# AtomGradient/swift-qwen3-tts

Hardware: AMD Instinct MI355X
Metric: codec_tokens_per_s (higher is better)
Workload: dtype bf16

## Files before the change

### swift-qwen3-tts_amd/csrc/engine.cc

```cpp
#include "engine.h"

#include <algorithm>
#include <cctype>
#include <chrono>
#include <cmath>
#include <cstdio>
#include <deque>
#include <functional>
#include <thread>

#include "codec.h"
#include "frontend.h"

namespace q3 {

namespace {
std::string lower(const std::string& s) {
    std::string o = s;
    for (auto& c : o) c = char(std::tolower((unsigned char)c));
    return o;
}
const char* const kCodecRangeMsg =
    "Audio decoding failed: the codec decoder produced a non-finite waveform -- also on the fp32 matrix-core convolutions (the "
    "reference's range), which a row is re-decoded on when it leaves the fp16 range of the default two-plane kernels";
// ... 27 lines not shown
    {
        int least = 0, greatest = 0;
        Q3_HIP(hipDeviceGetStreamPriorityRange(&least, &greatest));
        Q3_HIP(hipStreamCreateWithPriority(&st_, hipStreamNonBlocking, greatest));
        Q3_HIP(hipStreamCreateWithPriority(&st_codec_, hipStreamNonBlocking, least));
        hipDeviceProp_t prop{};
        Q3_HIP(hipGetDeviceProperties(&prop, m_->device));
        int cus = prop.multiProcessorCount / 2;
        if (opts.codec_overlap_cus > 0) cus = opts.codec_overlap_cus;
        else if (opts.codec_overlap_cus < 0) cus = 0;
        cus = std::min(cus, prop.multiProcessorCount) / 8 * 8;
        if (cus > 0 && cus < prop.multiProcessorCount) st_codec_part_ = masked_stream(cus, prop.multiProcessorCount);
    }
    for (auto& J : jobs_) {
        for (auto& e : J.ev_codec) Q3_HIP(hipEventCreate(&e));
        Q3_HIP(hipEventCreate(&J.ev_begin));
        Q3_HIP(hipEventCreate(&J.ev_first_audio));
        std::memset(J.nf_host.grow(size_t(std::max(opts.max_batch, 1))), 0, size_t(std::max(opts.max_batch, 1)) * 4);
    }
    for (auto& e : ev_) Q3_HIP(hipEventCreate(&e));
    for (auto& e : burst_ev_) Q3_HIP(hipEventCreateWithFlags(&e, hipEventDisableTiming));
    for (auto& e : ev_fe_) Q3_HIP(hipEventCreate(&e));
    Q3_HIP(hipEventCreateWithFlags(&fe_uploaded_, hipEventDisableTiming));
    Bm_ = opts.max_batch;
    Mp_ = std::getenv("Q3TTS_ROWS_64") ? 64 : std::max(256, 16 * int(align_up(size_t(opts.max_batch), 16)));
    Pcap_ = opts.max_prompt;
    Tcap_ = opts.max_prompt;
    Fcap_ = opts.max_frames;
    max_pages_ = ceil_div(Pcap_ + Fcap_ + 1, kPageTokens);
    n_pages_ = Bm_ * max_pages_;
    for (auto& kv : m_->cfg.talker.spk_id) speakers.push_back(kv.first);
    std::sort(speakers.begin(), speakers.end());
    alloc_workspace();
    if (std::getenv("Q3TTS_FRAME_STAMPS")) {
        Q3_HIP(hipMalloc(reinterpret_cast<void**>(&stamps_), 64 * 8));
        Q3_HIP(hipMemset(stamps_, 0, 64 * 8));
    }
    if (m_->has_codec) codec_ = std::make_unique<CodecRunner>(*m_, st_codec_, opts.codec_fp32 != 0);
    if (m_->has_codec_encoder || m_->has_speaker_encoder) fe_ = std::make_unique<VoiceFrontEnd>(*m_, st_);
}

hipStream_t Engine::masked_stream(int cus, int total) {
    std::vector<uint32_t> mask(size_t(ceil_div(total, 32)), 0u);
    for (int i = 0; i < cus; ++i) mask[size_t(i / 32)] |= 1u << (i % 32);
    hipStream_t st = nullptr;
    Q3_HIP(hipExtStreamCreateWithCUMask(&st, uint32_t(mask.size()), mask.data()));
    return st;
}

void Engine::prepare_job_pair() {
    job_chains = 2;
    if (opts_.codec_overlap_cus != 0 || !st_codec_part_ || st_codec_wide_) return;
    hipDeviceProp_t prop{};
    Q3_HIP(hipGetDeviceProperties(&prop, m_->device));
    st_codec_wide_ = masked_stream(prop.multiProcessorCount * 3 / 4 / 8 * 8, prop.multiProcessorCount);
}

Engine::~Engine() {
    if (worker_.joinable()) {
        {
            std::lock_guard<std::mutex> lk(work_mu_);
            work_stop_ = true;
        }
        work_cv_.notify_all();
        worker_.join();
    }
// ... 49 lines not shown
    if (st_) (void)hipStreamDestroy(st_);
}

void Engine::build_cp_proj_tables() {
    if (cp_tables_ || !m_->has_cp_proj || std::getenv("Q3TTS_NO_PROJ_TABLES")) return;
    const TalkerConfig& t = m_->cfg.talker;
    const int H = t.hidden_size, CH = m_->cp.hidden, MBL = Mp_ / 16, Vc = t.cp.vocab_size, nss = CH / 16;
    const int ntab = t.num_code_groups - 2;
    if (ntab <= 0) return;
    std::lock_guard<std::mutex> lock(m_->lazy_mutex);
    if (m_->cp_pe.empty()) {
        for (int i = 0; i < ntab; ++i) {
            uint16_t* pe = nullptr;
            float* pss = nullptr;
            Q3_HIP(hipMalloc(reinterpret_cast<void**>(&pe), size_t(Vc) * CH * 2));
            m_->lazy_allocs.push_back(pe);
            Q3_HIP(hipMalloc(reinterpret_cast<void**>(&pss), size_t(Vc) * nss * 4));
            m_->lazy_allocs.push_back(pss);
            for (int c0 = 0; c0 < Vc; c0 += Mp_) {
                const int rows = std::min(Mp_, Vc - c0);
                launch_tile_rows(m_->cp_emb[size_t(i)] + size_t(c0) * H, H, cp_x_, MBL, rows, H, st_);
                GemmArgs p = gemm_args(m_->cp_proj, cp_x_, rows);
                p.epi = 3; p.y = cp_.h; p.yMB = MBL; p.resid = 0; p.ss_out = cp_.ss_a;
                launch_gemm_skinny(p, st_);
                launch_untile_rows(cp_.h, MBL, pe + size_t(c0) * CH, CH, rows, CH, st_);
                launch_ss_to_table(cp_.ss_a, Mp_, pss + size_t(c0) * nss, nss, rows, st_);
            }
            m_->cp_pe.push_back(pe);
            m_->cp_pss.push_back(pss);
        }
        Q3_HIP(hipStreamSynchronize(st_));
    }
    cp_tables_ = true;
}

void Engine::alloc_workspace() {
    const TalkerConfig& t = m_->cfg.talker;
    const int H = t.hidden_size, CH = t.cp.hidden_size, TH = t.text_hidden_size;
    const int qd = t.num_attention_heads * kHeadDim, kd = t.num_key_value_heads * kHeadDim;
    const int cqd = t.cp.num_attention_heads * kHeadDim, ckd = t.cp.num_key_value_heads * kHeadDim;
    const int L = t.num_hidden_layers, CL = t.cp.num_hidden_layers;
    kv_layer_stride_ = size_t(n_pages_) * t.num_key_value_heads * kPageTokens * kHeadDim;
    cp_kv_layer_stride_ = size_t(Bm_) * t.cp.num_key_value_heads * kPageTokens * kHeadDim;
    proj_cap_ = Bm_ * (2 * Pcap_ + 8);
    for (int pass = 0; pass < 2; ++pass) {
        Bump b{pass ? ws_ : nullptr};
        Bump& x = b;
        auto stream = [&](Stream& s, int hid, int q, int k, int inter_p, int vocab) {
            s.ld_qkv = q + 2 * k;
            s.ld_act = inter_p;
            s.ld_logits = vocab;
            s.h = x.take<uint16_t>(size_t(Mp_) * hid);
            s.xn = x.take<uint16_t>(size_t(Mp_) * hid);
            s.ss_a = x.take<float>(size_t(hid / 16) * Mp_);
            s.ss_b = x.take<float>(size_t(hid / 16) * Mp_);
            s.qkv = x.take<uint16_t>(size_t(Mp_) * s.ld_qkv);
            s.ao = x.take<uint16_t>(size_t(Mp_) * q);
            s.act = x.take<uint16_t>(size_t(Mp_) * inter_p);
            s.logits = b.take<uint16_t>(size_t(Mp_) * vocab);
        };
        stream(tk_, H, qd, kd, m_->talker.max_inter_p, t.vocab_size);
        stream(cp_, CH, cqd, ckd, m_->cp.max_inter_p, t.cp.vocab_size);
        cp_x_ = x.take<uint16_t>(size_t(Mp_) * H);
        cp_x2_ = x.take<uint16_t>(size_t(Mp_) * H);
        cp_ss2_ = x.take<float>(size_t(Mp_));
        kpool_ = b.take<uint16_t>(kv_layer_stride_ * L);
// ... 20 lines not shown
        sp_dev_ = b.take<SamplingParams>(size_t(Bm_));
        ids_dev_ = b.take<int32_t>(size_t(proj_cap_));
        proj_in_ = b.take<uint16_t>(size_t(64) * TH);
        proj_mid_ = b.take<uint16_t>(size_t(64) * TH);
        proj_out_ = b.take<uint16_t>(size_t(proj_cap_ + 64) * H);
        compose_a_ = b.take<int32_t>(size_t(3) * Bm_ * (Pcap_ + Tcap_));
        compose_b_ = nullptr;
        if (!pass) {
            ws_bytes_ = align_up(b.off, 256);
            Q3_HIP(hipMalloc(reinterpret_cast<void**>(&ws_), ws_bytes_));
            Q3_HIP(hipMemset(ws_, 0, ws_bytes_));
        }
    }
    std::vector<int32_t> cbt((size_t)(Bm_));
    for (int i = 0; i < Bm_; ++i) cbt[size_t(i)] = i;
    Q3_HIP(hipMemcpy(cp_block_table_, cbt.data(), cbt.size() * 4, hipMemcpyHostToDevice));
}

GemmArgs Engine::gemm_args(const LinearW& L, const uint16_t* x, int M) const {
    GemmArgs a{};
    a.W = L.w;
    a.Wsb = L.sb;
    a.x = x;
    a.xMB = Mp_ / 16;
    a.M = M;
    a.Mpad = int(align_up(size_t(M), 16));
    a.N = L.Np;
    a.K = L.Kp;
    a.bias = L.bias;
    a.ss_ld = Mp_;
    return a;
}

void Engine::enqueue_layers(const StackW& s, Stream& w, int B, uint16_t* kpool, uint16_t* vpool, size_t layer_stride,
                            const int32_t* block_table, int max_pages, const int32_t* kv_len, const uint8_t* active,
                            int ss_count_in, int fixed_len, int chunk, const int32_t* chunk_n_prompt, int chunk_r_base) {
    const int H = s.hidden, MBL = Mp_ / 16, tiles = H / 16;
    const int M = B * (chunk > 1 ? chunk : 1);
    Q3_CHECK(M <= Mp_, 7, "internal error: chunk does not fit the activation buffers");
    const bool row_norm = M > 64;
    const bool prologue_qkv = H <= 2048 && !row_norm, prologue_mlp = H <= 2048 && !row_norm;
    const bool nt_off = debug_env().nt_off;
    const bool is_talker = &s == &m_->talker;
    const int ntw = is_talker && !nt_off ? 1 : 0;
    const int ntkv = ntw;
    auto norm_into_xn = [&](const uint16_t* nw, const float* ss, int ss_count) {
        NormRowsArgs n{};
        n.h = w.h; n.hMB = MBL; n.w = nw; n.eps = s.eps; n.out = w.xn; n.outMB = MBL; n.M = M; n.H = H;
        if (row_norm && H <= 2048) { n.ss_in = ss; n.ss_count = ss_count; n.ss_ld = Mp_; }
        launch_norm_rows(n, counted());
    };
    for (size_t l = 0; l < s.layers.size(); ++l) {
        const LayerW& L = s.layers[l];
        if (!prologue_qkv) norm_into_xn(L.ln1, w.ss_a, (l == 0) ? ss_count_in : tiles);
        GemmArgs q = gemm_args(L.qkv, prologue_qkv ? w.h : w.xn, M);
        q.epi = 0; q.y = w.qkv; q.ldy = w.ld_qkv; q.nt_weights = ntw;
        if (prologue_qkv) {
            q.norm_w = L.ln1; q.ss_in = w.ss_a; q.ss_count = (l == 0) ? ss_count_in : tiles; q.norm_dim = H; q.norm_eps = s.eps;
        }
        AttnArgs at{};
        at.qkv = w.qkv; at.ld = w.ld_qkv; at.qn_w = L.qn; at.kn_w = L.kn; at.eps = s.eps;
        at.rope_cos = s.rope_cos; at.rope_sin = s.rope_sin;
        at.kpool = kpool + l * layer_stride; at.vpool = vpool + l * layer_stride;
        at.block_table = block_table; at.max_pages = max_pages; at.kv_len = kv_len; at.active = active;
        at.out = w.ao; at.outMB = MBL; at.n_heads = s.n_heads; at.n_kv = s.n_kv; at.B = B;
        at.fixed_len = fixed_len; at.identity_pages = fixed_len >= 0 ? 1 : 0;
        at.chunk = chunk; at.chunk_n_prompt = chunk_n_prompt; at.chunk_r_base = chunk_r_base;
        at.scale = powf(float(kHeadDim), -0.5f);
        at.nt_kv = ntkv;
        launch_gemm_skinny(q, counted());
        launch_attn_decode(at, counted());
        GemmArgs o = gemm_args(L.o, w.ao, M);
        o.epi = 3; o.y = w.h; o.yMB = MBL; o.resid = 1; o.ss_out = w.ss_b; o.nt_weights = ntw;
        launch_gemm_skinny(o, counted());
        if (!prologue_mlp) norm_into_xn(L.ln2, w.ss_b, tiles);
        GemmArgs g = gemm_args(L.gateup, prologue_mlp ? w.h : w.xn, M);
        g.epi = 2; g.y = w.act; g.yMB = MBL; g.nt_weights = ntw;
        if (prologue_mlp) {
            g.norm_w = L.ln2; g.ss_in = w.ss_b; g.ss_count = tiles; g.norm_dim = H; g.norm_eps = s.eps;
        }
        launch_gemm_skinny(g, counted());
        GemmArgs d = gemm_args(L.down, w.act, M);
        d.epi = 3; d.y = w.h; d.yMB = MBL; d.resid = 1; d.ss_out = w.ss_a; d.nt_weights = ntw;
        launch_gemm_skinny(d, counted());
    }
}

void Engine::enqueue_talker_step(int B, bool with_head) {
    (void)with_head;
    enqueue_layers(m_->talker, tk_, B, kpool_, vpool_, kv_layer_stride_, block_table_, max_pages_, kv_len_, active_, 1, -1, 1, nullptr, 0);
}

void Engine::enqueue_cp_pass(int B, bool from_talker, int head, int cp_pos, bool projected) {
    const TalkerConfig& t = m_->cfg.talker;
    const int H = t.hidden_size, CH = m_->cp.hidden, MBL = Mp_ / 16;
    int ss_count = 1;
    auto talker_norm_into = [&](uint16_t* dst, float* ss_out) {
        NormRowsArgs n{};
        n.h = tk_.h; n.hMB = MBL; n.w = m_->talker.final_norm; n.eps = m_->talker.eps;
        n.out = dst; n.outMB = MBL; n.ss_out = ss_out; n.M = B; n.H = H;
        launch_norm_rows(n, counted());
    };
    if (m_->has_cp_proj && projected) {
        ss_count = CH / 16;
    } else if (m_->has_cp_proj) {
        if (from_talker) talker_norm_into(cp_x2_, nullptr);
        GemmArgs p = gemm_args(m_->cp_proj, from_talker ? cp_x2_ : cp_x_, B);
        p.epi = 3; p.y = cp_.h; p.yMB = MBL; p.resid = 0; p.ss_out = cp_.ss_a;
        launch_gemm_skinny(p, counted());
        ss_count = CH / 16;
    } else if (from_talker) {
        talker_norm_into(cp_.h, cp_.ss_a);
    }
    enqueue_layers(m_->cp, cp_, B, cp_kpool_, cp_vpool_, cp_kv_layer_stride_, cp_block_table_, 1, cp_len_, nullptr, ss_count, cp_pos, 1, nullptr, 0);
}

void Engine::enqueue_frame(int B, const DebugOpts* dbg) {
    struct Count {
        Engine* e;
        int B;
        ~Count() { e->frame_launches_[B] = e->launches_; }
    } count{this, B};
    launches_ = 0;
    const TalkerConfig& t = m_->cfg.talker;
    const int H = t.hidden_size, V = t.vocab_size, Vc = t.cp.vocab_size, CH = t.cp.hidden_size;
    const int groups = t.num_code_groups, MBL = Mp_ / 16;
    stamp(0);
    enqueue_talker_step(B, true);
    stamp(1);
    uint16_t* next_x = m_->has_cp_proj ? cp_x_ : cp_.h;
    float* next_ss = m_->has_cp_proj ? nullptr : cp_.ss_a;
    const bool pair = 2 * B <= Mp_;
    {
        GemmArgs hd = gemm_args(m_->codec_head, tk_.h, B);
        hd.epi = 0; hd.y = tk_.logits; hd.ldy = tk_.ld_logits;
        hd.norm_w = m_->talker.final_norm; hd.ss_in = tk_.ss_a; hd.ss_count = H / 16; hd.norm_dim = H; hd.norm_eps = m_->talker.eps;
        bool rode = false;
        if (pair) {
            NormRowsArgs n{};
            n.h = tk_.h; n.hMB = MBL; n.w = m_->talker.final_norm; n.eps = m_->talker.eps;
            n.out = next_x; n.outMB = MBL; n.ss_out = next_ss; n.M = B; n.H = H;
            rode = launch_gemm_skinny_with_norm_rows(hd, n, st_);
            if (rode) ++launches_;
            else launch_norm_rows(n, counted());
        }
        if (!rode) launch_gemm_skinny(hd, counted());
    }
// ... 14 lines not shown
    sa.logits_dump = (dbg && dbg->talker_logits) ? tl_dump_ : nullptr; sa.dump_ld = V; sa.dump_off = 0;
    sa.row_key = frame_row_key_;
    if (pair) {
        launch_sampler(sa, counted());
        int ss_count = 1;
        if (m_->has_cp_proj) {
            GemmArgs p = gemm_args(m_->cp_proj, cp_x_, 2 * B);
            p.epi = 3; p.y = cp_.h; p.yMB = MBL; p.resid = 0; p.ss_out = cp_.ss_a;
            launch_gemm_skinny(p, counted());
            ss_count = CH / 16;
        }
        stamp(2);
        enqueue_layers(m_->cp, cp_, B, cp_kpool_, cp_vpool_, cp_kv_layer_stride_, cp_block_table_, 1, cp_len_, nullptr, ss_count, 0, 2,
                       nullptr, 0);
        stamp(3);
    } else {
        launch_sampler(sa, counted());
        enqueue_cp_pass(B, true, -1, 0);
        if (!m_->has_cp_proj) {
            launch_copy_rows(cp_x2_, 0, cp_.h, 0, 1, Mp_ * H, counted());
            launch_copy_rows(reinterpret_cast<const uint16_t*>(cp_ss2_), 0, reinterpret_cast<uint16_t*>(cp_.ss_a), 0, 1, Mp_ * 2, counted());
        }
    }
    FrameEndArgs fe{};
    fe.cur_codes = cur_codes_; fe.codec_emb = m_->codec_emb; fe.cp_emb = m_->cp_emb_dev;
    fe.trailing = trailing_; fe.n_trailing = n_trailing_; fe.trailing_idx = trailing_idx_; fe.Tmax = Tcap_;
    fe.tts_pad = tts_pad_; fe.h = tk_.h; fe.hMB = MBL; fe.ss_out = tk_.ss_a; fe.H = H; fe.B = B; fe.groups = groups;
    fe.n_frames = n_frames_; fe.max_frames = max_frames_; fe.finished = finished_; fe.active = active_; fe.cp_len = cp_len_;
    bool fe_done = false;
    for (int i = 0; i < groups - 1; ++i) {
        const bool second_of_pair = pair && i == 0;
        const int Mh = second_of_pair ? 2 * B : B;
        if (!second_of_pair) {
            enqueue_cp_pass(B, false, i, i + 1, cp_tables_ && i >= 1);
            stamp(5);
        }
        {
            GemmArgs lh = gemm_args(m_->lm_head[size_t(i)], cp_.h, Mh);
            lh.epi = 0; lh.y = cp_.logits; lh.ldy = cp_.ld_logits;
            lh.norm_w = m_->cp.final_norm; lh.ss_in = cp_.ss_a; lh.ss_count = CH / 16; lh.norm_dim = CH; lh.norm_eps = m_->cp.eps;
            launch_gemm_skinny(lh, counted());
        }
        SamplerArgs sc{};
        sc.logits = cp_.logits + (second_of_pair ? size_t(B) * cp_.ld_logits : 0); sc.ldl = cp_.ld_logits; sc.V = Vc; sc.sp = sp_dev_;
        sc.is_talker = 0;
        sc.eos_id = -1; sc.cb = i + 1; sc.n_frames = n_frames_; sc.max_frames = max_frames_;
        sc.finished = finished_; sc.active = active_; sc.kv_len = cp_len_; sc.advance = 1; sc.advance_gate = nullptr;
        sc.cur_codes = cur_codes_; sc.codes = codes_; sc.Fmax = Fcap_;
        sc.forced = dbg ? forced_dev_ : nullptr; sc.forced_frames = dbg ? dbg->frames : 0;
        sc.sampled = dbg ? sampled_dev_ : nullptr;
        if (i + 1 < groups - 1) {
            sc.emb = m_->cp_emb[size_t(i)]; sc.emb_ld = H; sc.next_x = next_x; sc.next_MB = MBL; sc.next_ss = next_ss;
        }
        sc.H = H; sc.B = B;
        if (cp_tables_ && i + 1 < groups - 1) {
            sc.emb = m_->cp_pe[size_t(i)]; sc.emb_ld = CH; sc.H = CH; sc.next_x = cp_.h;
            sc.emb_ss = m_->cp_pss[size_t(i)]; sc.nss = CH / 16; sc.next_ss = cp_.ss_a; sc.next_ss_ld = Mp_;
        }
        sc.logits_dump = (dbg && dbg->cp_logits) ? cl_dump_ : nullptr; sc.dump_ld = (groups - 1) * Vc; sc.dump_off = i * Vc;
        sc.row_key = frame_row_key_;
        if (i == groups - 2 && Vc <= 2048) {
            launch_sampler_with_frame_end(sc, fe, counted());
            fe_done = true;
        } else {
            launch_sampler(sc, counted());
        }
        stamp(second_of_pair ? 4 : 6);
    }
    if (!fe_done) launch_frame_end(fe, counted());
    stamp(7);
}

hipGraphExec_t Engine::frame_graph(int B) {
    std::map<int, hipGraphExec_t>& graphs = frame_row_key_ ? qgraphs_ : graphs_;
    auto it = graphs.find(B);
    if (it != graphs.end()) return it->second;
    hipGraph_t g = nullptr;
    Q3_HIP(hipStreamBeginCapture(st_, hipStreamCaptureModeThreadLocal));
    try {
        enqueue_frame(B, nullptr);
    } catch (...) {
        (void)hipStreamEndCapture(st_, &g);
        if (g) (void)hipGraphDestroy(g);
        throw;
    }
    Q3_HIP(hipStreamEndCapture(st_, &g));
    hipGraphExec_t ge = nullptr;
    Q3_HIP(hipGraphInstantiate(&ge, g, nullptr, nullptr, 0));
    Q3_HIP(hipGraphDestroy(g));
    graphs[B] = ge;
// ... 888 lines not shown
    Q3_HIP(hipMemsetAsync(seen_, 0, size_t(n) * m_->cfg.talker.vocab_size, st_));
    Q3_HIP(hipMemsetAsync(codes_, 0, size_t(n) * Fcap_ * 16 * 4, st_));
    upload_sampling(sp, row_offset + sp.row_base, n);
    return Pmax;
}

void Engine::debug_buffers(int n, const DebugOpts& dbg) {
    const TalkerConfig& t = m_->cfg.talker;
    const int V = t.vocab_size, Vc = t.cp.vocab_size;
    for (void* p : {(void*)forced_dev_, (void*)sampled_dev_, (void*)tl_dump_, (void*)cl_dump_})
        if (p) (void)hipFree(p);
    forced_dev_ = sampled_dev_ = nullptr;
    tl_dump_ = cl_dump_ = nullptr;
    const size_t nf = size_t(n) * dbg.frames;
    if (dbg.forced_codes) {
        for (size_t i = 0; i < nf * 16; ++i) {
            const int32_t c = dbg.forced_codes[i];
            Q3_CHECK(c >= 0 && c < ((i & 15) == 0 ? V : Vc), 3, "Invalid input: forced code outside its vocabulary");
        }
        Q3_HIP(hipMalloc(reinterpret_cast<void**>(&forced_dev_), nf * 16 * 4));
        Q3_HIP(hipMemcpy(forced_dev_, dbg.forced_codes, nf * 16 * 4, hipMemcpyHostToDevice));
    }
    Q3_HIP(hipMalloc(reinterpret_cast<void**>(&sampled_dev_), nf * 16 * 4));
    Q3_HIP(hipMemset(sampled_dev_, 0xff, nf * 16 * 4));
    if (dbg.talker_logits) Q3_HIP(hipMalloc(reinterpret_cast<void**>(&tl_dump_), nf * V * 2));
    if (dbg.cp_logits) Q3_HIP(hipMalloc(reinterpret_cast<void**>(&cl_dump_), nf * (t.num_code_groups - 1) * Vc * 2));
}

int Engine::frame_loop(Job& J, const std::vector<ResolvedRequest>& rr, const q3tts_sampling& sp, q3tts_event_cb cb, void* user,
                       const DebugOpts* dbg, StreamedDecode& sd) {
    const int n = J.n;
    const bool use_graph = opts_.use_graph && !dbg;
    build_cp_proj_tables();
    hipGraphExec_t ge = use_graph ? frame_graph(n) : nullptr;
    int frames_cap = 0;
    for (auto& r : rr) frames_cap = std::max(frames_cap, r.max_frames);
    std::vector<int32_t> h_nframes((size_t)(n), 0);
    std::vector<uint8_t> h_fin((size_t)(n), 0);
    std::vector<int> reported((size_t)(n), 0);
    int launched = 0;
    const bool fixed_len = sp.force_frames > 0 || dbg;
    const int burst_frames = std::max(1, max_inflight_frames / job_chains / 2);
    hipEvent_t ring[2] = {burst_ev_[0], burst_ev_[1]};
    int bursts = 0;
    bool done = false;
    while (!done && launched < frames_cap) {
        if (bursts >= 2) Q3_HIP(hipEventSynchronize(ring[bursts & 1]));
        int burst = std::min(burst_frames, frames_cap - launched);
        if (sd.on) {
            const int need = std::min(frames_cap, sd.next_need(launched, sp.audio_chunk_frames, std::max(0, sp.audio_lookahead_frames)));
            if (need > launched) burst = std::min(burst, need - launched);
        }
        for (int i = 0; i < burst; ++i) {
            if (use_graph) Q3_HIP(hipGraphLaunch(ge, st_));
            else enqueue_frame(n, dbg);
        }
        launched += burst;
        if (!(fixed_len && !cb)) {
            Q3_HIP(hipMemcpyAsync(h_nframes.data(), n_frames_, size_t(n) * 4, hipMemcpyDeviceToHost, st_));
            Q3_HIP(hipMemcpyAsync(h_fin.data(), finished_, size_t(n), hipMemcpyDeviceToHost, st_));
        }
        Q3_HIP(hipEventRecord(ring[bursts & 1], st_));
        ++bursts;
        if (fixed_len && !cb) {
            if (sd.on) {
                for (int b = 0; b < n; ++b) sd.avail[size_t(b)] = std::min(launched, rr[size_t(b)].max_frames);
// ... 653 lines not shown
    launch_admit_rows(a, k, st_);
    Q3_HIP(hipEventRecord(ev_[1], st_));
    const double now = now_s();
    for (int j = 0; j < k; ++j) {
        sl[size_t(slots[size_t(j)])] = QSlot{idx[size_t(j)], 0, 0, np[size_t(j)], now, rr[size_t(j)].max_frames};
        live[idx[size_t(j)]].rr = std::move(rr[size_t(j)]);
    }
    return k;
}

void Engine::run_queued(QueueShared& q, int S, const q3tts_sampling& sp, q3tts_event_cb cb, void* user) {
    Q3_HIP(hipSetDevice(m_->device));
    Q3_CHECK(S >= 1 && S <= Bm_, 3, "Invalid input: slots must be between 1 and max_batch");
    Q3_CHECK(!job_outstanding(), 3, "Invalid input: a q3tts_generate_begin job is outstanding (q3tts_generate_end must be called first)");
    ensure_queue_ws();
    {
        if (q.voice_ref_max >= 0) extra_.grow(size_t(S) * (1 + q.voice_ref_max) * m_->cfg.talker.hidden_size);
    }
    const double t_call = now_s();
    std::vector<int32_t> bt(size_t(S) * max_pages_);
    for (size_t i = 0; i < bt.size(); ++i) bt[i] = int32_t(i);
    Q3_HIP(hipMemcpyAsync(block_table_, bt.data(), bt.size() * 4, hipMemcpyHostToDevice, st_));
    for (int32_t* p : {kv_len_, cp_len_, n_frames_, max_frames_, trailing_idx_, n_trailing_, n_prompt_})
        Q3_HIP(hipMemsetAsync(p, 0, size_t(S) * 4, st_));
    Q3_HIP(hipMemsetAsync(row_key_, 0, size_t(S) * 4, st_));
    Q3_HIP(hipMemsetAsync(active_, 0, size_t(S), st_));
    Q3_HIP(hipMemsetAsync(finished_, 1, size_t(S), st_));
    {
        q3tts_sampling call_wide = sp;
        call_wide.per_request = nullptr;
        upload_sampling(call_wide, 0u, S);
    }
    build_cp_proj_tables();
    struct KeyScope {
        Engine* e;
        ~KeyScope() { e->frame_row_key_ = nullptr; }
    } key_scope{this};
    frame_row_key_ = row_key_;
    hipGraphExec_t ge = opts_.use_graph ? frame_graph(S) : nullptr;
    Q3_HIP(hipStreamSynchronize(st_));

    std::vector<QSlot> sl((size_t)(S));
    std::unordered_map<int, QLive> live;
    std::vector<int> settled;
    std::deque<int> waiting;
    int dec = -1;
    struct DecodeGuard {
        Engine* e;
        int* dec;
        ~DecodeGuard() {
            if (*dec < 0) return;
            (void)hipEventSynchronize(e->jobs_[*dec].ev_codec[1]);
            e->release_job(e->jobs_[*dec]);
        }
    } dec_guard{this, &dec};
    double codec_ms = 0;
    auto deliver = [&](bool wait) {
        if (!wait) {
            std::lock_guard<std::mutex> lk(stage_mu_);
            if (jobs_[dec].stage == 1) return;
        }
        const int j = dec;
        dec = -1;
        const std::vector<int> batch = jobs_[j].req_index;
        end(j, nullptr);
        codec_ms += timing.codec_ms;
// ... 1268 lines not shown
```

### swift-qwen3-tts_amd/csrc/engine.h

```cpp
#pragma once
#include <atomic>
#include <cstdlib>
#include <map>
#include <memory>
#include <condition_variable>
#include <mutex>
#include <thread>
#include <string>
#include <unordered_map>
#include <vector>

#include "../../include/q3tts.h"
#include "kernels.h"
#include "model.h"
#include "session_queue.h"

namespace q3 {

struct DebugOpts {
    const int32_t* forced_codes = nullptr;
    int frames = 0;
    uint16_t* talker_logits = nullptr;
    uint16_t* cp_logits = nullptr;
    int32_t* sampled = nullptr;
// ... 162 lines not shown
    Model* m_;
  public:
    uint32_t row_offset = 0;
    std::mutex* cb_mutex = nullptr;
    int request_base = 0;
    int max_inflight_frames = 16;
    int job_chains = 1;
  private:
    q3tts_load_opts opts_;
    hipStream_t st_ = nullptr;
    hipStream_t st_codec_ = nullptr;
    hipStream_t st_codec_part_ = nullptr;
    hipStream_t st_codec_wide_ = nullptr;
    hipStream_t masked_stream(int cus, int total);
    hipStream_t codec_stream(bool overlapped, bool wide = false);
    hipEvent_t ev_[4] = {nullptr, nullptr, nullptr, nullptr};
    hipEvent_t burst_ev_[2] = {nullptr, nullptr};
    hipEvent_t ev_fe_[2] = {nullptr, nullptr};
    hipEvent_t fe_uploaded_ = nullptr;
    int Bm_ = 0, Mp_ = 0;
    int Pcap_ = 0, Tcap_ = 0, Fcap_ = 0, max_pages_ = 0, n_pages_ = 0;

    uint8_t* ws_ = nullptr;
    size_t ws_bytes_ = 0;
    struct Stream {
        uint16_t *h, *xn, *qkv, *ao, *act, *logits;
        float *ss_a, *ss_b;
        int ld_qkv, ld_act, ld_logits;
    } tk_{}, cp_{};
    uint16_t* cp_x_ = nullptr;
    uint16_t* cp_x2_ = nullptr;
    bool cp_tables_ = false;
    void build_cp_proj_tables();
    float* cp_ss2_ = nullptr;
    uint16_t *kpool_ = nullptr, *vpool_ = nullptr, *cp_kpool_ = nullptr, *cp_vpool_ = nullptr;
    size_t kv_layer_stride_ = 0, cp_kv_layer_stride_ = 0;
    int32_t *block_table_ = nullptr, *cp_block_table_ = nullptr;
    int32_t *kv_len_ = nullptr, *cp_len_ = nullptr, *n_frames_ = nullptr, *max_frames_ = nullptr;
    int32_t *trailing_idx_ = nullptr, *n_trailing_ = nullptr, *n_prompt_ = nullptr, *cur_codes_ = nullptr, *codes_ = nullptr;
    uint8_t *active_ = nullptr, *finished_ = nullptr, *seen_ = nullptr;
    uint16_t *prompt_ = nullptr, *trailing_ = nullptr, *tts_pad_ = nullptr;
    SamplingParams* sp_dev_ = nullptr;
    int32_t* ids_dev_ = nullptr;
    uint16_t *proj_in_ = nullptr, *proj_mid_ = nullptr, *proj_out_ = nullptr;
    int proj_cap_ = 0;
    int32_t *compose_a_ = nullptr, *compose_b_ = nullptr;
    int32_t *forced_dev_ = nullptr, *sampled_dev_ = nullptr;
    uint16_t *tl_dump_ = nullptr, *cl_dump_ = nullptr;

    struct Job {
        std::atomic<bool> busy{false};
        uint64_t seq = 0;
        std::vector<ResolvedRequest> rr;
        std::vector<int> np;
        q3tts_sampling sp{};
        bool overlapped = false;
        bool frontend = false;
        bool background = false;
        int back = 0;
        int back_status = 0;
        std::string back_err;
        int n = 0, Fdec = 0, up = 0;
        std::vector<int> frames, ref_T, target_tokens, n_prompt;
        std::vector<int> req_index;
        std::vector<q3tts_result*> row_out;
        std::vector<double> row_span;
// ... 73 lines not shown
    const float* upload_audio(const float* audio, int64_t n);
    bool prepare_clone_rows(std::vector<ResolvedRequest>& reqs);

    void alloc_workspace();
    ResolvedRequest resolve(const q3tts_request& r, const q3tts_sampling& sp, const Voice* voice = nullptr) const;
    void check_reference(const float* ref_audio, int64_t n_ref_samples, const int32_t* ref_text_ids, int n_ref_text_ids) const;
    int open_job(const q3tts_request* reqs, int n, const q3tts_sampling& sp, const DebugOpts* dbg, std::vector<ResolvedRequest>& rr,
                 double& t_start, const Voice* const* voices);
    int reserve_rows(const std::vector<ResolvedRequest>& rr, const std::vector<int>& np, const std::vector<int>& nt,
                     const q3tts_sampling& sp);
    void debug_buffers(int n, const DebugOpts& dbg);
    struct StreamedDecode;
    struct SlotStream;
    int frame_loop(Job& J, const std::vector<ResolvedRequest>& rr, const q3tts_sampling& sp, q3tts_event_cb cb, void* user,
                   const DebugOpts* dbg, StreamedDecode& sd);
    void hand_off(Job& J, const std::vector<ResolvedRequest>& rr, StreamedDecode& sd, int launched, bool overlapped);
    void back_half(Job& J, const std::vector<ResolvedRequest>& rr, const std::vector<int>& np, const q3tts_sampling& sp,
                   q3tts_event_cb cb, void* user, const DebugOpts* dbg, bool streamed, bool overlapped, double t_start);
    void worker_loop();
    std::thread worker_;
    std::mutex work_mu_;
    std::condition_variable work_cv_;
    Job* work_ = nullptr;
    bool work_stop_ = false;
    void job_timing(Job& J, const std::vector<int>& np, int launched);
    void upload_sampling(const q3tts_sampling& sp, uint32_t row0, int n);
    int64_t kv_bytes(int n_prompt, int frames) const;
    int launches_per_step(int B) const;
    void assemble_prompts(const std::vector<ResolvedRequest>& reqs, std::vector<int>& n_prompt, std::vector<int>& n_trailing,
                          const std::vector<int>* trailing_rows = nullptr);
    void enqueue_prefill(Stream& w, int n, int Pmax, const int32_t* block_table, int32_t* kv_len, const int32_t* n_prompt,
                         uint8_t* active);
    void project_rows(const std::vector<int32_t>& ids, int rows);
    void enqueue_layers(const StackW& s, Stream& w, int B, uint16_t* kpool, uint16_t* vpool, size_t layer_stride,
                        const int32_t* block_table, int max_pages, const int32_t* kv_len, const uint8_t* active,
                        int ss_count_in, int fixed_len, int chunk, const int32_t* chunk_n_prompt, int chunk_r_base);
    void enqueue_talker_step(int B, bool with_head);
    void enqueue_cp_pass(int B, bool from_talker, int head, int cp_pos, bool projected = false);
    void enqueue_frame(int B, const DebugOpts* dbg);
    hipGraphExec_t frame_graph(int B);
    const uint32_t* frame_row_key_ = nullptr;
    std::map<int, hipGraphExec_t> qgraphs_;
    uint8_t* qws_ = nullptr;
    Stream qk_{};
    int32_t *q_bt_ = nullptr, *q_kv_len_ = nullptr, *q_n_prompt_ = nullptr;
    uint8_t* q_active_ = nullptr;
    AdmitDesc* q_desc_ = nullptr;
    std::vector<AdmitDesc> q_desc_host_;
    uint32_t* row_key_ = nullptr;
    std::vector<int32_t> q_host_;
    void ensure_queue_ws();
    struct QSlot {
        int req = -1;
        int since = 0;
        int reported = 0;
        int np = 0;
        double t0 = 0;
        int cap = 0;
    };
    struct QLive;
    int admit(QueueShared& q, std::vector<QSlot>& sl, std::unordered_map<int, QLive>& live);
    void cancel_slots(uint64_t mask, int slots);
    GemmArgs gemm_args(const LinearW& L, const uint16_t* x, int M) const;
};


class Session;

class EngineGroup {
  public:
    EngineGroup(std::unique_ptr<Model> model, const q3tts_load_opts& opts);
// ... 90 lines not shown
```

### swift-qwen3-tts_amd/csrc/kernels.h

```cpp
#pragma once
#include <hip/hip_runtime.h>

#include <cstdint>

namespace q3 {

struct DebugEnv {
    bool gemm_no_row_split;
    bool gemm_one_pair;
    bool no_tall_gemm;
    int tall_shape;
    int chunk_qsplit;
    bool conv_no_pw;
    bool nt_off;
    bool serial_jobs;
    bool fail_back_half;
    bool no_prefix_cache;
};
const DebugEnv& debug_env();
void debug_env_reload();

constexpr int kPageTokens = 64;
constexpr int kHeadDim = 128;

// ... 106 lines not shown
    const uint16_t* logits;
    int ldl, V;
    const SamplingParams* sp;
    int is_talker;
    int suppress_lo, suppress_hi, eos_id;
    uint8_t* seen;
    int cb;
    const int32_t* n_frames;
    const int32_t* max_frames;
    uint8_t* finished;
    uint8_t* active;
    int32_t* kv_len;
    int advance;
    const uint8_t* advance_gate;
    int32_t* cur_codes;
    int32_t* codes;
    int Fmax;
    const int32_t* forced;
    int forced_frames;
    int32_t* sampled;
    const uint16_t* emb;
    int emb_ld;
    uint16_t* next_x;
    int next_MB;
    int next_row0;
    float* next_ss;
    const float* emb_ss;
    int nss, next_ss_ld;
    int H;
    int B;
    uint16_t* logits_dump;
    int dump_ld, dump_off;
    const uint32_t* row_key;
};
void launch_sampler(const SamplerArgs& a, hipStream_t st);
void launch_sampler_with_frame_end(const SamplerArgs& a, const FrameEndArgs& fe, hipStream_t st);
void launch_ss_to_table(const float* ss, int ss_ld, float* dst, int nss, int rows, hipStream_t st);

void launch_gather_rows(const uint16_t* table, int ld, const int32_t* ids, const int32_t* token_map,
                        int n, int dim, uint16_t* out, int ldo, int out_MB, hipStream_t st);
void launch_tile_rows(const uint16_t* src, int lds, uint16_t* dst, int dstMB, int rows, int dim, hipStream_t st);
void launch_untile_rows(const uint16_t* src, int srcMB, uint16_t* dst, int ldd, int rows, int dim, hipStream_t st);
void launch_add_rows(const uint16_t* a, int lda, const uint16_t* b, int ldb, int rows, int dim,
                     uint16_t* out, int ldo, hipStream_t st);

struct PrefillLoadArgs {
    const uint16_t* prompt;
    const int32_t* n_prompt;
    int Pmax, step, H, B;
    uint16_t* h;
    int hMB;
    float* ss_out;
    uint8_t* active;
};
void launch_prefill_load(const PrefillLoadArgs& a, hipStream_t st);
void launch_advance_len(int32_t* kv_len, const uint8_t* active, int B, hipStream_t st);
void launch_stamp(unsigned long long* acc, unsigned long long* last, int k, hipStream_t st);
void launch_prefill_chunk_load(const PrefillLoadArgs& a, int C, hipStream_t st);
void launch_advance_len_chunk(int32_t* kv_len, const int32_t* n_prompt, int r_base, int C, int B, hipStream_t st);

struct AdmitDesc {
    int32_t slot, n_trailing, max_frames;
    uint32_t row_key;
    SamplingParams sp;
};
struct AdmitArgs {
    const AdmitDesc* desc;
    const uint16_t* src_h;
// ... 35 lines not shown
```

### swift-qwen3-tts_amd/csrc/kernels/sampler.hip

```cpp
#include "../common.h"
#include "../kernels.h"
#include "row_jobs.h"

namespace q3 {
namespace {

constexpr int kMaxVAll = 4096;

__device__ __forceinline__ void philox4x32_10(uint32_t c0, uint32_t c1, uint32_t c2, uint32_t c3, uint32_t k0,
                                              uint32_t k1, uint32_t (&out)[4]) {
#pragma unroll
    for (int r = 0; r < 10; ++r) {
        const uint64_t p0 = (uint64_t)0xD2511F53u * c0;
        const uint64_t p1 = (uint64_t)0xCD9E8D57u * c2;
        const uint32_t n0 = (uint32_t)(p1 >> 32) ^ c1 ^ k0;
        const uint32_t n1 = (uint32_t)p1;
        const uint32_t n2 = (uint32_t)(p0 >> 32) ^ c3 ^ k1;
        const uint32_t n3 = (uint32_t)p0;
        c0 = n0; c1 = n1; c2 = n2; c3 = n3;
        k0 += 0x9E3779B9u;
        k1 += 0xBB67AE85u;
    }
    out[0] = c0; out[1] = c1; out[2] = c2; out[3] = c3;
}
// ... 75 lines not shown
        float a, b, c, d;
        if constexpr (O == 32) { XorPartner::swap32(x.v, a, b); XorPartner::swap32(fi, c, d); }
        else { XorPartner::swap16(x.v, a, b); XorPartner::swap16(fi, c, d); }
        const bool upper = O == 32 ? ((threadIdx.x & 32) != 0) : ((threadIdx.x & 16) != 0);
        y.v = upper ? a : b;
        y.i = __float_as_int(upper ? c : d);
    } else if constexpr (O == 8) {
        y.v = XorPartner::x8(x.v); y.i = __float_as_int(XorPartner::x8(fi));
    } else if constexpr (O == 4) {
        y.v = XorPartner::x4(x.v); y.i = __float_as_int(XorPartner::x4(fi));
    } else if constexpr (O == 2) {
        y.v = XorPartner::x2(x.v); y.i = __float_as_int(XorPartner::x2(fi));
    } else {
        y.v = XorPartner::x1(x.v); y.i = __float_as_int(XorPartner::x1(fi));
    }
    return y;
}

template <int kThreads>
__device__ Best block_argmax(Best x, Best* scratch) {
    x = better(x, partner<32>(x));
    x = better(x, partner<16>(x));
    x = better(x, partner<8>(x));
    x = better(x, partner<4>(x));
    x = better(x, partner<2>(x));
    x = better(x, partner<1>(x));
    const int wave = threadIdx.x >> 6;
    __syncthreads();
    if ((threadIdx.x & 63) == 0) scratch[wave] = x;
    __syncthreads();
    Best r = scratch[0];
    for (int w = 1; w < kThreads / 64; ++w) r = better(r, scratch[w]);
    return r;
}

template <int kThreads, int kMaxV, bool TALKER, bool FEND>
__device__ __forceinline__ void sampler_body(const SamplerArgs& a, const FrameEndArgs* fe) {
    constexpr int kElems = kMaxV / kThreads;
    __builtin_amdgcn_s_setprio(3);
    __shared__ float vals[kMaxV];
    __shared__ uint32_t sortbuf[kMaxV];
    __shared__ float sval[kMaxV];
    __shared__ int n_surv;
    __shared__ uint32_t hist[2][256];
    __shared__ Best scratch[kThreads / 64];
    __shared__ uint32_t wcount[kElems][kThreads / 64];
    __shared__ int sel[2][2];

    const int b = blockIdx.x, tid = threadIdx.x;
    const int V = a.V;
    const uint16_t* lrow = a.logits + (size_t)b * a.ldl;
    uint16_t raw[kElems];
    uint8_t was_seen[kElems];
    const bool want_seen = TALKER && a.seen;
#pragma unroll
    for (int k = 0; k < kElems; ++k) {
        const int i = k * kThreads + tid;
        const int ic = i < V ? i : V - 1;
        raw[k] = lrow[ic];
        was_seen[k] = want_seen ? a.seen[(size_t)b * V + ic] : (uint8_t)0;
    }
    const SamplingParams sp = a.sp[b];
    const bool row_done = a.finished[b] != 0;
    const int frame = a.n_frames[b];
    const uint8_t gate_raw = *(a.advance_gate ? a.advance_gate + b : a.finished + b);
    const uint32_t key_raw = *(a.row_key ? a.row_key + b : reinterpret_cast<const uint32_t*>(a.n_frames) + b);
// ... 192 lines not shown
            }
        }
        __syncthreads();
        const int ns = n_surv;
        Best x{-INFINITY, 0x7fffffff};
        for (int q = tid; q < ns; q += kThreads) {
            const int i = (int)sortbuf[q];
            const float v = rbf(sval[q] * invt) + gumbel_noise(sp.seed, row_key, draw, (uint32_t)i);
            x = better(x, Best{v, i});
        }
        Best r = block_argmax<kThreads>(x, scratch);
        tok = (r.i == 0x7fffffff) ? 0 : r.i;
    }

    int used = tok;
    if (a.forced && frame < a.forced_frames) used = a.forced[((size_t)b * a.forced_frames + frame) * 16 + a.cb];
    if (tid == 0) {
        if (a.sampled && frame < a.forced_frames) a.sampled[((size_t)b * a.forced_frames + frame) * 16 + a.cb] = tok;
        a.cur_codes[(size_t)b * 16 + a.cb] = used;
        if (TALKER) {
            if (a.seen && used >= 0 && used < V) a.seen[(size_t)b * V + used] = 1;
            if (a.advance && a.active[b]) a.kv_len[b] += 1;
            if (used == a.eos_id) {
                a.finished[b] = 1;
                a.active[b] = 0;
            } else if (frame < a.Fmax) {
                a.codes[((size_t)b * a.Fmax + frame) * 16] = used;
            }
        } else {
            if (a.advance && gate) a.kv_len[b] += 1;
            if (frame < a.Fmax) a.codes[((size_t)b * a.Fmax + frame) * 16 + a.cb] = used;
        }
    }
    if (a.next_x) {
        const uint4* src = reinterpret_cast<const uint4*>(a.emb + (size_t)used * a.emb_ld);
        float ss = 0.f;
        for (int i = tid; i < a.H / 8; i += kThreads) {
            const uint4 v = src[i];
            const uint32_t w[4] = {v.x, v.y, v.z, v.w};
#pragma unroll
            for (int j = 0; j < 4; ++j) ss += lo_bf(w[j]) * lo_bf(w[j]) + hi_bf(w[j]) * hi_bf(w[j]);
            *reinterpret_cast<uint4*>(a.next_x + act_tiled_offset(b + a.next_row0, 8 * i, a.next_MB)) = v;
        }
        if (a.emb_ss) {
            for (int j = tid; j < a.nss; j += kThreads)
                a.next_ss[(size_t)j * a.next_ss_ld + b + a.next_row0] = a.emb_ss[(size_t)used * a.nss + j];
        } else if (a.next_ss) {
            ss = wave_sum(ss);
            __syncthreads();
            if ((tid & 63) == 0) vals[tid >> 6] = ss;
            __syncthreads();
            if (tid == 0) {
                float t = 0.f;
                for (int w = 0; w < kThreads / 64; ++w) t += vals[w];
                a.next_ss[b] = t;
            }
        }
    }
    if constexpr (FEND) {
        __shared__ float fe_sh[4];
        frame_end_job(*fe, b, tid, used, fe_sh);
    }
}

template <int kThreads, int kMaxV, bool TALKER>
__global__ __launch_bounds__(kThreads) void sampler_kernel(SamplerArgs a) {
    sampler_body<kThreads, kMaxV, TALKER, false>(a, nullptr);
}
struct SamplerFendArgs {
    SamplerArgs s;
    FrameEndArgs fe;
};
__global__ __launch_bounds__(1024) void sampler_fend_kernel(SamplerFendArgs a) {
    sampler_body<1024, 2048, false, true>(a.s, &a.fe);
}

}

void launch_sampler_with_frame_end(const SamplerArgs& a, const FrameEndArgs& fe, hipStream_t st) {
    Q3_CHECK(!a.is_talker && a.V <= 2048, 3, "sampler: the end-of-frame rider belongs to a code-predictor draw");
    SamplerFendArgs s{a, fe};
    hipLaunchKernelGGL(sampler_fend_kernel, dim3(a.B), dim3(1024), 0, st, s);
}

void launch_sampler(const SamplerArgs& a, hipStream_t st) {
    Q3_CHECK(a.V <= kMaxVAll, 3, "sampler: vocabulary larger than 4096 is not supported");
    if (!a.is_talker && a.V <= 2048) hipLaunchKernelGGL((sampler_kernel<1024, 2048, false>), dim3(a.B), dim3(1024), 0, st, a);
    else if (a.is_talker) hipLaunchKernelGGL((sampler_kernel<1024, 4096, true>), dim3(a.B), dim3(1024), 0, st, a);
    else hipLaunchKernelGGL((sampler_kernel<1024, 4096, false>), dim3(a.B), dim3(1024), 0, st, a);
}

}
```

### swift-qwen3-tts_amd/csrc/model.h

```cpp
#pragma once
#include <memory>
#include <mutex>
#include <string>
#include <vector>

#include "config.h"
#include "safetensors.h"

namespace q3 {

struct LinearW {
    const uint16_t* w = nullptr;
    const uint32_t* sb = nullptr;
    const uint16_t* bias = nullptr;
    int N = 0, K = 0;
    int Np = 0, Kp = 0;
};

struct LayerW {
    const uint16_t* ln1 = nullptr;
    const uint16_t* ln2 = nullptr;
    const uint16_t* qn = nullptr;
    const uint16_t* kn = nullptr;
    LinearW qkv;
// ... 118 lines not shown
        int C = 0;
    };
    Block blocks[3];
    ConvW mfa, asp_tdnn, asp_conv, fc;
    int scale = 8, enc_dim = 0;
};

struct Model {
    ModelConfig cfg;
    int device = 0;
    uint8_t* arena = nullptr;
    size_t arena_bytes = 0;

    StackW talker, cp;
    const uint16_t* codec_emb = nullptr;
    const uint16_t* text_emb = nullptr;
    const int32_t* token_map = nullptr;
    int64_t text_emb_rows = 0;
    LinearW fc1, fc2, codec_head, cp_proj;
    bool has_cp_proj = false;
    std::vector<LinearW> lm_head;
    std::vector<const uint16_t*> cp_emb;
    const uint16_t* const* cp_emb_dev = nullptr;
    bool has_codec = false;
    CodecW codec;
    bool has_codec_encoder = false;
    CodecEncW codec_enc;
    bool has_speaker_encoder = false;
    SpeakerEncW speaker;
    int64_t step_weight_bytes = 0;
    std::vector<void*> side_allocs;
    mutable std::vector<const uint16_t*> cp_pe;
    mutable std::vector<const float*> cp_pss;
    mutable std::vector<void*> lazy_allocs;
    mutable std::mutex lazy_mutex;

    ~Model();
};

struct LoadOptions {
    int device = 0;
    int max_pos_talker = 4096;
    bool skip_tensor_data = false;
};

std::unique_ptr<Model> load_model(const std::string& dir, const LoadOptions& opt);

void launch_tile_weights(const uint16_t* src, int N, int K, uint16_t* dst, int KC, int tile_off, int tile_stride,
                         hipStream_t st, int rows_per_tile = 16, int row_off = 0);
void launch_tile_int4(const uint32_t* wq, const uint16_t* scales, const uint16_t* biases, int N, int K, void* dq,
                      uint32_t* dsb, int KC, int tile_off, int tile_stride, hipStream_t st, int rows_per_tile = 16, int row_off = 0);

}
```

Before: 10350.

## Precompute code-predictor layer-0 QKV per code and gather it in the sampler

The first code-predictor layer's QKV depends only on the sampled code (embedding, optional projection, RMSNorm, QKV GEMM), so the change precomputes a per-codebook table of layer-0 QKV rows for every vocabulary entry. The sampler then copies the chosen row straight into the QKV buffer, and layer 0's QKV GEMM and norm are skipped in CP passes after the first. This removes one skinny GEMM launch and its weight read per CP step. In exchange it costs extra device memory (vocab x qkv width per codebook) and a one-time table build, and it can be turned off with an environment variable.

```diff
diff --git a/swift-qwen3-tts_amd/csrc/engine.cc b/swift-qwen3-tts_amd/csrc/engine.cc
--- a/swift-qwen3-tts_amd/csrc/engine.cc
+++ b/swift-qwen3-tts_amd/csrc/engine.cc
@@ -83,6 +83,7 @@
     for (auto& kv : m_->cfg.talker.spk_id) speakers.push_back(kv.first);
     std::sort(speakers.begin(), speakers.end());
     alloc_workspace();
+    cp_qkv_off_ = std::getenv("Q3TTS_NO_QKV_TABLES") != nullptr;
     if (std::getenv("Q3TTS_FRAME_STAMPS")) {
         Q3_HIP(hipMalloc(reinterpret_cast<void**>(&stamps_), 64 * 8));
         Q3_HIP(hipMemset(stamps_, 0, 64 * 8));
@@ -198,6 +199,46 @@
         Q3_HIP(hipStreamSynchronize(st_));
     }
     cp_tables_ = true;
+}
+
+void Engine::set_cp_gather(SamplerArgs& sc, int i) const {
+    const int H = m_->cfg.talker.hidden_size, CH = m_->cp.hidden;
+    sc.next_MB = Mp_ / 16;
+    if (cp_tables_) {
+        sc.emb = m_->cp_pe[size_t(i)]; sc.emb_ld = CH; sc.H = CH; sc.next_x = cp_.h;
+        sc.emb_ss = m_->cp_pss[size_t(i)]; sc.nss = CH / 16; sc.next_ss = cp_.ss_a; sc.next_ss_ld = Mp_;
+    } else {
+        sc.emb = m_->cp_emb[size_t(i)]; sc.emb_ld = H; sc.H = H;
+        sc.next_x = m_->has_cp_proj ? cp_x_ : cp_.h; sc.next_ss = m_->has_cp_proj ? nullptr : cp_.ss_a;
+    }
+}
+
+void Engine::build_cp_qkv_tables() {
+    if (cp_qkv_tables_ || cp_qkv_off_ || (m_->has_cp_proj && !cp_tables_)) return;
+    const TalkerConfig& t = m_->cfg.talker;
+    const int CH = m_->cp.hidden, Vc = t.cp.vocab_size, ld = cp_.ld_qkv;
+    const int ntab = t.num_code_groups - 2;
+    if (ntab <= 0 || CH > 2048 || m_->cp.layers.empty()) return;
+    std::lock_guard<std::mutex> lock(m_->lazy_mutex);
+    if (m_->cp_qkv.empty()) {
+        const int blk = std::min(64, Mp_);
+        for (int i = 0; i < ntab; ++i) {
+            uint16_t* tab = nullptr;
+            Q3_HIP(hipMalloc(reinterpret_cast<void**>(&tab), size_t(Vc) * ld * 2));
+            m_->lazy_allocs.push_back(tab);
+            SamplerArgs g{};
+            set_cp_gather(g, i);
+            for (int c0 = 0; c0 < Vc; c0 += blk) {
+                const int rows = std::min(blk, Vc - c0);
+                launch_gather_codes(g, c0, rows, st_);
+                launch_gemm_skinny(qkv_gemm_args(m_->cp, 0, cp_, rows, true, cp_tables_ ? CH / 16 : 1, 0), st_);
+                launch_copy_rows(cp_.qkv, ld, tab + size_t(c0) * ld, ld, rows, ld, st_);
+            }
+            m_->cp_qkv.push_back(tab);
+        }
+        Q3_HIP(hipStreamSynchronize(st_));
+    }
+    cp_qkv_tables_ = true;
 }
 
 void Engine::alloc_workspace() {
@@ -284,9 +325,20 @@
     return a;
 }
 
+GemmArgs Engine::qkv_gemm_args(const StackW& s, size_t l, const Stream& w, int M, bool prologue, int ss_count, int ntw) const {
+    const LayerW& L = s.layers[l];
+    GemmArgs q = gemm_args(L.qkv, prologue ? w.h : w.xn, M);
+    q.epi = 0; q.y = w.qkv; q.ldy = w.ld_qkv; q.nt_weights = ntw;
+    if (prologue) {
+        q.norm_w = L.ln1; q.ss_in = w.ss_a; q.ss_count = ss_count; q.norm_dim = s.hidden; q.norm_eps = s.eps;
+    }
+    return q;
+}
+
 void Engine::enqueue_layers(const StackW& s, Stream& w, int B, uint16_t* kpool, uint16_t* vpool, size_t layer_stride,
                             const int32_t* block_table, int max_pages, const int32_t* kv_len, const uint8_t* active,
-                            int ss_count_in, int fixed_len, int chunk, const int32_t* chunk_n_prompt, int chunk_r_base) {
+                            int ss_count_in, int fixed_len, int chunk, const int32_t* chunk_n_prompt, int chunk_r_base,
+                            bool skip_qkv0) {
     const int H = s.hidden, MBL = Mp_ / 16, tiles = H / 16;
     const int M = B * (chunk > 1 ? chunk : 1);
     Q3_CHECK(M <= Mp_, 7, "internal error: chunk does not fit the activation buffers");
@@ -304,12 +356,9 @@
     };
     for (size_t l = 0; l < s.layers.size(); ++l) {
         const LayerW& L = s.layers[l];
-        if (!prologue_qkv) norm_into_xn(L.ln1, w.ss_a, (l == 0) ? ss_count_in : tiles);
-        GemmArgs q = gemm_args(L.qkv, prologue_qkv ? w.h : w.xn, M);
-        q.epi = 0; q.y = w.qkv; q.ldy = w.ld_qkv; q.nt_weights = ntw;
-        if (prologue_qkv) {
-            q.norm_w = L.ln1; q.ss_in = w.ss_a; q.ss_count = (l == 0) ? ss_count_in : tiles; q.norm_dim = H; q.norm_eps = s.eps;
-        }
+        const bool have_qkv = skip_qkv0 && l == 0;
+        if (!prologue_qkv && !have_qkv) norm_into_xn(L.ln1, w.ss_a, (l == 0) ? ss_count_in : tiles);
+        const GemmArgs q = qkv_gemm_args(s, l, w, M, prologue_qkv, (l == 0) ? ss_count_in : tiles, ntw);
         AttnArgs at{};
         at.qkv = w.qkv; at.ld = w.ld_qkv; at.qn_w = L.qn; at.kn_w = L.kn; at.eps = s.eps;
         at.rope_cos = s.rope_cos; at.rope_sin = s.rope_sin;
@@ -320,7 +369,7 @@
         at.chunk = chunk; at.chunk_n_prompt = chunk_n_prompt; at.chunk_r_base = chunk_r_base;
         at.scale = powf(float(kHeadDim), -0.5f);
         at.nt_kv = ntkv;
-        launch_gemm_skinny(q, counted());
+        if (!have_qkv) launch_gemm_skinny(q, counted());
         launch_attn_decode(at, counted());
         GemmArgs o = gemm_args(L.o, w.ao, M);
         o.epi = 3; o.y = w.h; o.yMB = MBL; o.resid = 1; o.ss_out = w.ss_b; o.nt_weights = ntw;
@@ -343,7 +392,7 @@
     enqueue_layers(m_->talker, tk_, B, kpool_, vpool_, kv_layer_stride_, block_table_, max_pages_, kv_len_, active_, 1, -1, 1, nullptr, 0);
 }
 
-void Engine::enqueue_cp_pass(int B, bool from_talker, int head, int cp_pos, bool projected) {
+void Engine::enqueue_cp_pass(int B, bool from_talker, int head, int cp_pos, bool projected, bool skip_qkv0) {
     const TalkerConfig& t = m_->cfg.talker;
     const int H = t.hidden_size, CH = m_->cp.hidden, MBL = Mp_ / 16;
     int ss_count = 1;
@@ -364,7 +413,8 @@
     } else if (from_talker) {
         talker_norm_into(cp_.h, cp_.ss_a);
     }
-    enqueue_layers(m_->cp, cp_, B, cp_kpool_, cp_vpool_, cp_kv_layer_stride_, cp_block_table_, 1, cp_len_, nullptr, ss_count, cp_pos, 1, nullptr, 0);
+    enqueue_layers(m_->cp, cp_, B, cp_kpool_, cp_vpool_, cp_kv_layer_stride_, cp_block_table_, 1, cp_len_, nullptr, ss_count, cp_pos, 1, nullptr, 0,
+                   skip_qkv0);
 }
 
 void Engine::enqueue_frame(int B, const DebugOpts* dbg) {
@@ -445,7 +495,7 @@
         const bool second_of_pair = pair && i == 0;
         const int Mh = second_of_pair ? 2 * B : B;
         if (!second_of_pair) {
-            enqueue_cp_pass(B, false, i, i + 1, cp_tables_ && i >= 1);
+            enqueue_cp_pass(B, false, i, i + 1, cp_tables_ && i >= 1, cp_qkv_tables_ && i >= 1);
             stamp(5);
         }
         {
@@ -462,13 +512,13 @@
         sc.cur_codes = cur_codes_; sc.codes = codes_; sc.Fmax = Fcap_;
         sc.forced = dbg ? forced_dev_ : nullptr; sc.forced_frames = dbg ? dbg->frames : 0;
         sc.sampled = dbg ? sampled_dev_ : nullptr;
+        sc.H = H; sc.B = B;
         if (i + 1 < groups - 1) {
-            sc.emb = m_->cp_emb[size_t(i)]; sc.emb_ld = H; sc.next_x = next_x; sc.next_MB = MBL; sc.next_ss = next_ss;
-        }
-        sc.H = H; sc.B = B;
-        if (cp_tables_ && i + 1 < groups - 1) {
-            sc.emb = m_->cp_pe[size_t(i)]; sc.emb_ld = CH; sc.H = CH; sc.next_x = cp_.h;
-            sc.emb_ss = m_->cp_pss[size_t(i)]; sc.nss = CH / 16; sc.next_ss = cp_.ss_a; sc.next_ss_ld = Mp_;
+            set_cp_gather(sc, i);
+            if (cp_qkv_tables_) {
+                sc.qkv_tab = m_->cp_qkv[size_t(i)]; sc.qkv_ld = cp_.ld_qkv; sc.qkv_out = cp_.qkv;
+                sc.emb_ss = nullptr; sc.next_ss = nullptr;
+            }
         }
         sc.logits_dump = (dbg && dbg->cp_logits) ? cl_dump_ : nullptr; sc.dump_ld = (groups - 1) * Vc; sc.dump_off = i * Vc;
         sc.row_key = frame_row_key_;
@@ -1423,6 +1473,7 @@
     const int n = J.n;
     const bool use_graph = opts_.use_graph && !dbg;
     build_cp_proj_tables();
+    build_cp_qkv_tables();
     hipGraphExec_t ge = use_graph ? frame_graph(n) : nullptr;
     int frames_cap = 0;
     for (auto& r : rr) frames_cap = std::max(frames_cap, r.max_frames);
@@ -2142,6 +2193,7 @@
         upload_sampling(call_wide, 0u, S);
     }
     build_cp_proj_tables();
+    build_cp_qkv_tables();
     struct KeyScope {
         Engine* e;
         ~KeyScope() { e->frame_row_key_ = nullptr; }
diff --git a/swift-qwen3-tts_amd/csrc/engine.h b/swift-qwen3-tts_amd/csrc/engine.h
--- a/swift-qwen3-tts_amd/csrc/engine.h
+++ b/swift-qwen3-tts_amd/csrc/engine.h
@@ -218,6 +218,10 @@
     uint16_t* cp_x2_ = nullptr;
     bool cp_tables_ = false;
     void build_cp_proj_tables();
+    bool cp_qkv_off_ = false;
+    bool cp_qkv_tables_ = false;
+    void build_cp_qkv_tables();
+    void set_cp_gather(SamplerArgs& sc, int i) const;
     float* cp_ss2_ = nullptr;
     uint16_t *kpool_ = nullptr, *vpool_ = nullptr, *cp_kpool_ = nullptr, *cp_vpool_ = nullptr;
     size_t kv_layer_stride_ = 0, cp_kv_layer_stride_ = 0;
@@ -357,11 +361,13 @@
     void enqueue_prefill(Stream& w, int n, int Pmax, const int32_t* block_table, int32_t* kv_len, const int32_t* n_prompt,
                          uint8_t* active);
     void project_rows(const std::vector<int32_t>& ids, int rows);
+    GemmArgs qkv_gemm_args(const StackW& s, size_t l, const Stream& w, int M, bool prologue, int ss_count, int ntw) const;
     void enqueue_layers(const StackW& s, Stream& w, int B, uint16_t* kpool, uint16_t* vpool, size_t layer_stride,
                         const int32_t* block_table, int max_pages, const int32_t* kv_len, const uint8_t* active,
-                        int ss_count_in, int fixed_len, int chunk, const int32_t* chunk_n_prompt, int chunk_r_base);
+                        int ss_count_in, int fixed_len, int chunk, const int32_t* chunk_n_prompt, int chunk_r_base,
+                        bool skip_qkv0 = false);
     void enqueue_talker_step(int B, bool with_head);
-    void enqueue_cp_pass(int B, bool from_talker, int head, int cp_pos, bool projected = false);
+    void enqueue_cp_pass(int B, bool from_talker, int head, int cp_pos, bool projected = false, bool skip_qkv0 = false);
     void enqueue_frame(int B, const DebugOpts* dbg);
     hipGraphExec_t frame_graph(int B);
     const uint32_t* frame_row_key_ = nullptr;
diff --git a/swift-qwen3-tts_amd/csrc/kernels.h b/swift-qwen3-tts_amd/csrc/kernels.h
--- a/swift-qwen3-tts_amd/csrc/kernels.h
+++ b/swift-qwen3-tts_amd/csrc/kernels.h
@@ -162,8 +162,12 @@
     uint16_t* logits_dump;
     int dump_ld, dump_off;
     const uint32_t* row_key;
+    const uint16_t* qkv_tab;
+    uint16_t* qkv_out;
+    int qkv_ld;
 };
 void launch_sampler(const SamplerArgs& a, hipStream_t st);
+void launch_gather_codes(const SamplerArgs& a, int code0, int rows, hipStream_t st);
 void launch_sampler_with_frame_end(const SamplerArgs& a, const FrameEndArgs& fe, hipStream_t st);
 void launch_ss_to_table(const float* ss, int ss_ld, float* dst, int nss, int rows, hipStream_t st);
 
diff --git a/swift-qwen3-tts_amd/csrc/kernels/sampler.hip b/swift-qwen3-tts_amd/csrc/kernels/sampler.hip
--- a/swift-qwen3-tts_amd/csrc/kernels/sampler.hip
+++ b/swift-qwen3-tts_amd/csrc/kernels/sampler.hip
@@ -131,6 +131,36 @@
     Best r = scratch[0];
     for (int w = 1; w < kThreads / 64; ++w) r = better(r, scratch[w]);
     return r;
+}
+
+template <int kThreads>
+__device__ __forceinline__ void gather_next_input(const SamplerArgs& a, const int b, const int used, float* red) {
+    const int tid = threadIdx.x;
+    if (a.next_x) {
+        const uint4* src = reinterpret_cast<const uint4*>(a.emb + (size_t)used * a.emb_ld);
+        float ss = 0.f;
+        for (int i = tid; i < a.H / 8; i += kThreads) {
+            const uint4 v = src[i];
+            const uint32_t w[4] = {v.x, v.y, v.z, v.w};
+#pragma unroll
+            for (int j = 0; j < 4; ++j) ss += lo_bf(w[j]) * lo_bf(w[j]) + hi_bf(w[j]) * hi_bf(w[j]);
+            *reinterpret_cast<uint4*>(a.next_x + act_tiled_offset(b + a.next_row0, 8 * i, a.next_MB)) = v;
+        }
+        if (a.emb_ss) {
+            for (int j = tid; j < a.nss; j += kThreads)
+                a.next_ss[(size_t)j * a.next_ss_ld + b + a.next_row0] = a.emb_ss[(size_t)used * a.nss + j];
+        } else if (a.next_ss) {
+            ss = wave_sum(ss);
+            __syncthreads();
+            if ((tid & 63) == 0) red[tid >> 6] = ss;
+            __syncthreads();
+            if (tid == 0) {
+                float t = 0.f;
+                for (int w = 0; w < kThreads / 64; ++w) t += red[w];
+                a.next_ss[b] = t;
+            }
+        }
+    }
 }
 
 template <int kThreads, int kMaxV, bool TALKER, bool FEND>
@@ -389,31 +419,14 @@
             if (frame < a.Fmax) a.codes[((size_t)b * a.Fmax + frame) * 16 + a.cb] = used;
         }
     }
-    if (a.next_x) {
-        const uint4* src = reinterpret_cast<const uint4*>(a.emb + (size_t)used * a.emb_ld);
-        float ss = 0.f;
-        for (int i = tid; i < a.H / 8; i += kThreads) {
-            const uint4 v = src[i];
-            const uint32_t w[4] = {v.x, v.y, v.z, v.w};
-#pragma unroll
-            for (int j = 0; j < 4; ++j) ss += lo_bf(w[j]) * lo_bf(w[j]) + hi_bf(w[j]) * hi_bf(w[j]);
-            *reinterpret_cast<uint4*>(a.next_x + act_tiled_offset(b + a.next_row0, 8 * i, a.next_MB)) = v;
-        }
-        if (a.emb_ss) {
-            for (int j = tid; j < a.nss; j += kThreads)
-                a.next_ss[(size_t)j * a.next_ss_ld + b + a.next_row0] = a.emb_ss[(size_t)used * a.nss + j];
-        } else if (a.next_ss) {
-            ss = wave_sum(ss);
-            __syncthreads();
-            if ((tid & 63) == 0) vals[tid >> 6] = ss;
-            __syncthreads();
-            if (tid == 0) {
-                float t = 0.f;
-                for (int w = 0; w < kThreads / 64; ++w) t += vals[w];
-                a.next_ss[b] = t;
-            }
-        }
-    }
+    const int nq = a.qkv_tab ? a.qkv_ld / 8 : 0;
+    const uint4* qsrc = reinterpret_cast<const uint4*>(a.qkv_tab + (size_t)used * a.qkv_ld);
+    uint4* qdst = reinterpret_cast<uint4*>(a.qkv_out + (size_t)b * a.qkv_ld);
+    uint4 q0 = make_uint4(0, 0, 0, 0);
+    if (tid < nq) q0 = qsrc[tid];
+    gather_next_input<kThreads>(a, b, used, vals);
+    if (tid < nq) qdst[tid] = q0;
+    for (int i = tid + kThreads; i < nq; i += kThreads) qdst[i] = qsrc[i];
     if constexpr (FEND) {
         __shared__ float fe_sh[4];
         frame_end_job(*fe, b, tid, used, fe_sh);
@@ -428,6 +441,10 @@
     SamplerArgs s;
     FrameEndArgs fe;
 };
+__global__ __launch_bounds__(1024) void gather_codes_kernel(SamplerArgs a, int code0) {
+    __shared__ float red[1024 / 64];
+    gather_next_input<1024>(a, blockIdx.x, code0 + blockIdx.x, red);
+}
 __global__ __launch_bounds__(1024) void sampler_fend_kernel(SamplerFendArgs a) {
     sampler_body<1024, 2048, false, true>(a.s, &a.fe);
 }
@@ -440,7 +457,13 @@
     hipLaunchKernelGGL(sampler_fend_kernel, dim3(a.B), dim3(1024), 0, st, s);
 }
 
+void launch_gather_codes(const SamplerArgs& a, int code0, int rows, hipStream_t st) {
+    Q3_CHECK(a.emb && a.next_x && rows > 0 && code0 >= 0, 3, "gather_codes: nothing to gather");
+    hipLaunchKernelGGL(gather_codes_kernel, dim3(rows), dim3(1024), 0, st, a, code0);
+}
+
 void launch_sampler(const SamplerArgs& a, hipStream_t st) {
+    Q3_CHECK(!a.qkv_tab || (a.qkv_out && a.qkv_ld % 8 == 0), 3, "sampler: q/k/v table without a destination");
     Q3_CHECK(a.V <= kMaxVAll, 3, "sampler: vocabulary larger than 4096 is not supported");
     if (!a.is_talker && a.V <= 2048) hipLaunchKernelGGL((sampler_kernel<1024, 2048, false>), dim3(a.B), dim3(1024), 0, st, a);
     else if (a.is_talker) hipLaunchKernelGGL((sampler_kernel<1024, 4096, true>), dim3(a.B), dim3(1024), 0, st, a);
diff --git a/swift-qwen3-tts_amd/csrc/model.h b/swift-qwen3-tts_amd/csrc/model.h
--- a/swift-qwen3-tts_amd/csrc/model.h
+++ b/swift-qwen3-tts_amd/csrc/model.h
@@ -174,6 +174,7 @@
     std::vector<void*> side_allocs;
     mutable std::vector<const uint16_t*> cp_pe;
     mutable std::vector<const float*> cp_pss;
+    mutable std::vector<const uint16_t*> cp_qkv;
     mutable std::vector<void*> lazy_allocs;
     mutable std::mutex lazy_mutex;
 
```

Result: slower. 10190 (-1.6%).
